# real-world-cryprography/APSU

Hardware: AMD Instinct MI355X
Metric: sender query-eval ms (ComputePowers + all BinBundles + gather), 16M-4096 params (lower is better)
Workload: dtype u64; 1 GPU; 16M-4096: n=8192, 4 bundle indices x 7 BinBundles (degrees [1303, 170]), 6 source -> 72 target powers, ps_low_degree=44; db_bytes_rank0=5459379072, binbundles_rank0=28, parallelism=binbundle-shard x1

## Files before the change

apsu_amd/csrc/engine_steps.cpp:

```cpp
#include "engine_impl.h"

#include <string>

namespace apsu_he {

namespace {

[[noreturn]] void refuse(const std::string &why) { throw std::invalid_argument("debug_run_step: " + why); }
void need(bool ok, const char *why) { if (!ok) refuse(why); }

void check_canonical(const u64 *x, size_t rows, const std::vector<u64> &mods, size_t n, const char *what)
{
    for (size_t r = 0; r < rows; r++) {
        const u64 m = mods[r % mods.size()], *row = x + r * n;
        u64 bad = 0;
        for (size_t k = 0; k < n; k++) bad |= (u64)(row[k] >= m);
        if (bad) refuse(std::string(what) + " holds a word that is not a canonical residue of its limb");
    }
}

}

void Engine::debug_run_step(const StepArgs &a)
{
    Enter g(this);
    TIER1_SLOTS();
    if (a.step == STEP_ROOTS_SPLIT) { debug_run_db_step(a); return; }
    if (a.step >= STEP_NTT_INFO) { debug_run_ntt_step(a); return; }
    if (a.step >= STEP_POLYN_WITH_ROOTS) { debug_run_db_step(a); return; }
    check_level(a.chain_idx);
    const LevelConstants &h = hlevel(a.chain_idx);
    const size_t n = hp_.n;
    const int L = h.L, nB = h.nB, nBsk = nB + 1, E = L + nBsk, K = hp_.K;
    const bool raw = a.flags & STEP_RAW, flag2 = a.flags & STEP_ACCUMULATE, store = a.flags & STEP_STORE, with_key = a.flags & STEP_KEY;
    const bool unrolled = behz_unrolled(L, nB);
    const std::vector<u64> q(h.q.begin(), h.q.end());
    std::vector<u64> bsk(h.B.begin(), h.B.end());
    bsk.push_back(h.m_sk);
    std::vector<u64> ext = q;
    ext.insert(ext.end(), bsk.begin(), bsk.end());
    const std::vector<u64> tmod{ hp_.t };
    const size_t batch = a.batch > 0 ? (size_t)a.batch : 0, polys = a.polys > 0 ? (size_t)a.polys : 0, terms = a.terms > 0 ? (size_t)a.terms : 0;

    if (a.step == STEP_LEVEL_INFO) {
        const size_t w = 4 + (size_t)L + nBsk + 2;
        need(a.out[0] && a.out_words[0] >= w, "level_info: out[0] too small");
        u64 *o = a.out[0];
        *o++ = (u64)L; *o++ = (u64)nB; *o++ = unrolled ? 1 : 0; *o++ = (u64)K;
        for (u64 v : q) *o++ = v;
        for (u64 v : bsk) *o++ = v;
        *o++ = hp_.using_keyswitching ? hp_.key_q[K - 1] : 0;
        *o++ = (u64)hp_.irrelevant_bit_count;
        return;
    }

    need(batch >= 1 && batch <= 64, "batch out of range (1 .. 64)");
    auto in_is = [&](int i, size_t words, const char *what) { if (!a.in[i] || a.in_words[i] != words) refuse(std::string(what) + ": wrong size"); };
    auto out_is = [&](int i, size_t words, const char *what) { if (!a.out[i] || a.out_words[i] != words) refuse(std::string(what) + ": wrong size"); };
    auto canon = [&](int i, const std::vector<u64> &mods, const char *what) { check_canonical(a.in[i], a.in_words[i] / n, mods, n, what); };
    auto canon_out = [&](int i, const std::vector<u64> &mods, const char *what) { check_canonical(a.out[i], a.out_words[i] / n, mods, n, what); };

    std::vector<FinishJob> fin;
    std::vector<FinishSumJob> fsum;
    std::vector<TensorJob> tj;
    std::vector<TensorConvJob> tcj;
    std::vector<TensorSumJob> tsj;
    std::vector<CtJob> cj;
    std::vector<SumJob> sj;
    std::vector<PlainJob> pj;
    std::vector<I0Job> ij;
    std::vector<EpiJob> ej;
    std::vector<unsigned char> flags8;

    WITH_ARENA({
        fin.clear(); fsum.clear(); tj.clear(); tcj.clear(); tsj.clear(); cj.clear(); sj.clear(); pj.clear(); ij.clear(); ej.clear();
        auto up = [&](const u64 *src, size_t words) {
            u64 *d = ws(words);
            HIP_CHECK(hipMemcpyAsync(d, src, words * sizeof(u64), hipMemcpyHostToDevice, st_));
            return d;
        };
        auto up_in = [&](int i) { return up(a.in[i], a.in_words[i]); };
        auto down = [&](int i, const u64 *src) { HIP_CHECK(hipMemcpyAsync(a.out[i], src, a.out_words[i] * sizeof(u64), hipMemcpyDeviceToHost, st_)); };
        auto jobs = [&](const auto &v) {
            using T = typename std::decay_t<decltype(v)>::value_type;
            T *d = ws_as<T>(v.size());
            HIP_CHECK(hipMemcpyAsync(d, v.data(), v.size() * sizeof(T), hipMemcpyHostToDevice, st_));
            return static_cast<const T *>(d);
        };

        switch (a.step) {
        case STEP_BEHZ_EXT: {
            need(polys >= 1 && polys <= 16, "behz_ext: polys out of range");
            need(!raw, "behz_ext: launch_behz_ext has no RAW form");
            in_is(0, batch * polys * L * n, "behz_ext: in[0] [batch][polys][L][n]");
            out_is(0, batch * polys * E * n, "behz_ext: out[0] [batch][polys][E][n]");
            canon(0, q, "behz_ext: in[0]");
            u64 *o = ws(a.out_words[0]);
            launch_behz_ext(dlevel(a.chain_idx), L, nB, up_in(0), polys * L * n, (int)polys, o, n, (int)batch, st_);
            down(0, o);
        } break;
        case STEP_DROP_BEHZ_EXT: {
            need(polys >= 1 && polys <= 16, "drop_behz_ext: polys out of range");
            need(a.chain_idx + 1 <= hp_.first_chain_idx, "drop_behz_ext: there is no level above chain_idx to drop from");
            need(unrolled, "drop_behz_ext: launch_drop_behz_ext exists for the unrolled sizes only (L == nB <= 3)");
            in_is(0, batch * polys * (L + 1) * n, "drop_behz_ext: in[0] [batch][polys][L + 1][n]");
            out_is(0, batch * polys * E * n, "drop_behz_ext: out[0] [batch][polys][E][n]");
            if (!raw) canon(0, hlevel(a.chain_idx + 1).q, "drop_behz_ext: in[0]");
            u64 *o = ws(a.out_words[0]);
            if (!launch_drop_behz_ext(dlevel(a.chain_idx), L, nB, up_in(0), polys * (L + 1) * n, (int)polys, o, n, (int)batch, st_, raw))
                throw std::logic_error("debug_run_step: launch_drop_behz_ext declined an unrolled level");
            down(0, o);
        } break;
        case STEP_TENSOR: {
            in_is(0, batch * 2 * E * n, "tensor: in[0] [batch][2][E][n]");
            in_is(1, batch * 2 * E * n, "tensor: in[1] [batch][2][E][n]");
            out_is(0, batch * 3 * E * n, "tensor: out[0] [batch][3][E][n]");
            canon(0, ext, "tensor: in[0]");
            canon(1, ext, "tensor: in[1]");
            const u64 *x = up_in(0), *y = up_in(1);
            u64 *o = ws(a.out_words[0]);
            for (size_t b = 0; b < batch; b++) tj.push_back(TensorJob{ x + b * 2 * E * n, y + b * 2 * E * n, o + b * 3 * E * n });
            launch_tensor(dlevel(a.chain_idx), jobs(tj), n, (int)batch, st_);
            down(0, o);
        } break;
        case STEP_TENSOR_CONV: {
            const size_t sa = polys, sb = terms;
            need(sa >= 1 && sb >= 1 && sa + sb - 1 <= CT_SIZE_MAX, "tensor_conv: sizes out of range (polys = sa, terms = sb, sa + sb - 1 <= 16)");
            in_is(0, batch * sa * E * n, "tensor_conv: in[0] [batch][sa][E][n]");
            in_is(1, batch * sb * E * n, "tensor_conv: in[1] [batch][sb][E][n]");
            out_is(0, batch * (sa + sb - 1) * E * n, "tensor_conv: out[0] [batch][sa + sb - 1][E][n]");
            canon(0, ext, "tensor_conv: in[0]");
            canon(1, ext, "tensor_conv: in[1]");
            const u64 *x = up_in(0), *y = up_in(1);
            u64 *o = ws(a.out_words[0]);
            for (size_t b = 0; b < batch; b++) tcj.push_back(TensorConvJob{ x + b * sa * E * n, y + b * sb * E * n, o + b * (sa + sb - 1) * E * n, (int)sa, (int)sb });
// ... 206 lines not shown
```

apsu_amd/csrc/kernels_behz.hip:

```cpp
#include "launch_behz.h"
#include "kernel_launch.h"
#include "eval_plan.h"

namespace apsu_he {

template <int TL, int TNB>
__global__ __launch_bounds__(EW_T) void k_behz_ext(const DevLevel *__restrict__ lv, const u64 *__restrict__ in,
                                                   size_t in_stride, int polys, u64 *__restrict__ out, size_t n)
{
    const size_t k = (size_t)blockIdx.x * EW_T + threadIdx.x;
    if (k >= n) return;
    const int L = TL ? TL : lv->L, nBsk = TL ? TNB + 1 : lv->nBsk, E = L + nBsk;
    constexpr int LMAX = TL ? TL : DMAXL;
    constexpr int BMAX = TL ? TNB + 1 : DMAXB;
    const size_t c = blockIdx.y / polys, p = blockIdx.y % polys;
    const u64 *src = in + c * in_stride + p * (size_t)L * n;
    u64 *dst = out + (size_t)blockIdx.y * E * n;
    u64 xs[LMAX];
    u32 mt_acc = 0;
#pragma unroll
    for (int j = 0; j < LMAX; j++) {
        if (TL || j < L) {
            const u64 x = src[(size_t)j * n + k];
            dst[(size_t)j * n + k] = x;
// ... 86 lines not shown
    }
    behz_ext2_body<TL>(lv, xin, dst, n, k);
}

bool launch_drop_behz_ext(const DevLevel *lv, int L, int nB, const u64 *in, size_t in_stride, int polys, u64 *out, size_t n, int cts,
                          hipStream_t st, bool raw)
{
    if (!cts) return true;
    const dim3 g = ew_grid(n, cts * polys), t(EW_T);
#define EXT2_CASE(TL) if (behz_unrolled(L, nB) && L == TL) { \
        if (raw) hipLaunchKernelGGL((k_behz_ext2<TL, true, true>), g, t, 0, st, lv, in, in_stride, polys, out, n); \
        else hipLaunchKernelGGL((k_behz_ext2<TL, true>), g, t, 0, st, lv, in, in_stride, polys, out, n); \
        KERNEL_CHECK(); return true; }
    EXT2_CASE(1) EXT2_CASE(2) EXT2_CASE(3)
#undef EXT2_CASE
    return false;
}

void launch_behz_ext(const DevLevel *lv, int L, int nB, const u64 *in, size_t in_stride, int polys, u64 *out, size_t n, int cts,
                     hipStream_t st)
{
    if (!cts) return;
    const dim3 g = ew_grid(n, cts * polys), t(EW_T);
#define EXT2_CASE(TL) if (behz_unrolled(L, nB) && L == TL) { hipLaunchKernelGGL((k_behz_ext2<TL, false>), g, t, 0, st, lv, in, in_stride, polys, out, n); KERNEL_CHECK(); return; }
    EXT2_CASE(1) EXT2_CASE(2) EXT2_CASE(3)
#undef EXT2_CASE
    if (L == 4 && nB == 4) hipLaunchKernelGGL((k_behz_ext<4, 4>), g, t, 0, st, lv, in, in_stride, polys, out, n);
    else hipLaunchKernelGGL((k_behz_ext<0, 0>), g, t, 0, st, lv, in, in_stride, polys, out, n);
    KERNEL_CHECK();
}

__global__ __launch_bounds__(EW_T) void k_tensor(const DevLevel *__restrict__ lv, const TensorJob *__restrict__ jobs, size_t n)
{
    const size_t k = (size_t)blockIdx.x * EW_T + threadIdx.x;
    if (k >= n) return;
    const TensorJob job = jobs[blockIdx.y];
    const int E = lv->E;
    const size_t ps = (size_t)E * n;
    for (int e = 0; e < E; e++) {
        const Mod m = lv->ext[e];
        const size_t o = e * n + k;
        const u64 a0 = job.a[o], a1 = job.a[ps + o], b0 = job.b[o], b1 = job.b[ps + o];
        job.d[o] = mulmod(a0, b0, m);
        u128p mid = mul128(a0, b1);
        mac128(mid, a1, b0);
        job.d[ps + o] = barrett128(mid, m);
        job.d[2 * ps + o] = mulmod(a1, b1, m);
    }
}

void launch_tensor(const DevLevel *lv, const TensorJob *jobs, size_t n, int batch, hipStream_t st)
{
    hipLaunchKernelGGL(k_tensor, ew_grid(n, batch), dim3(EW_T), 0, st, lv, jobs, n);
    KERNEL_CHECK();
}

__global__ __launch_bounds__(EW_T) void k_tensor_conv(const DevLevel *__restrict__ lv, const TensorConvJob *__restrict__ jobs, size_t n)
{
    const size_t k = (size_t)blockIdx.x * EW_T + threadIdx.x;
    if (k >= n) return;
    const TensorConvJob job = jobs[blockIdx.y];
    const int E = lv->E;
    const size_t ps = (size_t)E * n;
    const int so = job.sa + job.sb - 1;
    for (int e = 0; e < E; e++) {
        const Mod m = lv->ext[e];
        const size_t o = e * n + k;
        for (int I = 0; I < so; I++) {
            const int i0 = I - (job.sb - 1) > 0 ? I - (job.sb - 1) : 0, i1 = I < job.sa - 1 ? I : job.sa - 1;
            u64 acc = 0;
            for (int i = i0; i <= i1; i++) acc = addmod(acc, mulmod(job.a[i * ps + o], job.b[(I - i) * ps + o], m), m.q);
            job.d[I * ps + o] = acc;
        }
    }
}

void launch_tensor_conv(const DevLevel *lv, const TensorConvJob *jobs, size_t n, int njobs, hipStream_t st)
{
    if (!njobs) return;
    hipLaunchKernelGGL(k_tensor_conv, ew_grid(n, njobs), dim3(EW_T), 0, st, lv, jobs, n);
    KERNEL_CHECK();
}

__global__ __launch_bounds__(EW_T) void k_tensor_sum(const DevLevel *__restrict__ lv, const TensorSumJob *__restrict__ jobs, size_t n, int e0)
{
    const size_t k = (size_t)blockIdx.x * EW_T + threadIdx.x;
    if (k >= n) return;
    const TensorSumJob job = jobs[blockIdx.z];
    const int E = lv->E, L = lv->L, e = blockIdx.y + e0;
    const size_t ps = (size_t)E * n, o = (size_t)e * n + k;
    const Mod m = lv->ext[e];
    if (e < L) {
        for (int i = 0; i < job.terms; i++) {
            const u64 *a = job.a + (size_t)i * 2 * ps, *b = job.b + (size_t)i * 2 * ps;
            const u64 a0 = a[o], a1 = a[ps + o], b0 = b[o], b1 = b[ps + o];
            u64 *d = job.dq + (size_t)i * 3 * L * n + o;
            d[0] = mulmod(a0, b0, m);
            u128p mid = mul128(a0, b1);
            mac128(mid, a1, b0);
            d[(size_t)L * n] = barrett128(mid, m);
            d[(size_t)2 * L * n] = mulmod(a1, b1, m);
        }
    } else {
        u128p s0{ 0, 0 }, s1{ 0, 0 }, s2{ 0, 0 };
        u64 r0 = 0, r1 = 0, r2 = 0;
        for (int i = 0; i < job.terms; i++) {
            const u64 *a = job.a + (size_t)i * 2 * ps, *b = job.b + (size_t)i * 2 * ps;
            const u64 a0 = a[o], a1 = a[ps + o], b0 = b[o], b1 = b[ps + o];
            mac128(s0, a0, b0);
            mac128(s1, a0, b1);
            mac128(s1, a1, b0);
            mac128(s2, a1, b1);
            if ((i & 7) == 7 || i + 1 == job.terms) {
                r0 = addmod(r0, barrett128(s0, m), m.q);
                r1 = addmod(r1, barrett128(s1, m), m.q);
                r2 = addmod(r2, barrett128(s2, m), m.q);
                s0 = s1 = s2 = u128p{ 0, 0 };
            }
        }
        const int nBsk = E - L;
        u64 *d = job.bs + (size_t)(e - L) * n + k;
        d[0] = r0;
        d[(size_t)nBsk * n] = r1;
        d[(size_t)2 * nBsk * n] = r2;
    }
}

void launch_tensor_sum(const DevLevel *lv, int E, const TensorSumJob *jobs, size_t n, int njobs, int e0, hipStream_t st)
{
    if (!njobs || e0 >= E) return;
    hipLaunchKernelGGL(k_tensor_sum, dim3((unsigned)((n + EW_T - 1) / EW_T), E - e0, njobs), dim3(EW_T), 0, st, lv, jobs, n, e0);
    KERNEL_CHECK();
}

template <int TL, int TNB>
__device__ __forceinline__ void behz_finish_coeff(const DevLevel *__restrict__ lv, const u64 *__restrict__ dq, size_t term_stride,
                                                  int terms, const u64 *__restrict__ dbsk, size_t n, u64 *res )
{
    const int L = TL ? TL : lv->L, nB = TL ? TNB : lv->nB, nBsk = nB + 1;
    constexpr int LMAX = TL ? TL : DMAXL;
    constexpr int BMAX = TL ? TNB + 1 : DMAXB;
    u64 xq[LMAX];
#pragma unroll
    for (int j = 0; j < LMAX; j++) xq[j] = 0;
    for (int it = 0; it < terms; it++) {
#pragma unroll
        for (int j = 0; j < LMAX; j++)
            if (TL || j < L) xq[j] += mul_shoup(dq[it * term_stride + (size_t)j * n], lv->t_inv_punct_q[j].w, lv->t_inv_punct_q[j].wq, lv->q[j].q);
    }
    u64 ys[BMAX];
    u64 fl_sk = 0;
#pragma unroll
    for (int i = 0; i < BMAX; i++) {
        if (TL || i < nBsk) {
            const Mod m = lv->bsk[i];
            u128p acc{ 0, 0 };
#pragma unroll
            for (int j = 0; j < LMAX; j++)
                if (TL || j < L) mac128(acc, xq[j], lv->q_to_bsk[i][j]);
            const u64 conv = barrett128(acc, m);
            const u64 xb = mul_shoup(dbsk[(size_t)i * n], lv->t_bsk[i].w, lv->t_bsk[i].wq, m.q);
            const u64 fl = mul_shoup(xb + (m.q - conv), lv->inv_prod_q_bsk[i].w, lv->inv_prod_q_bsk[i].wq, m.q);
            if (i < nB) ys[i] = mul_shoup(fl, lv->inv_punct_B[i].w, lv->inv_punct_B[i].wq, m.q);
            else fl_sk = fl;
        }
    }
    const Mod msk = lv->bsk[nB];
    u128p acc{ 0, 0 };
#pragma unroll
    for (int i = 0; i < BMAX - 1; i++)
        if (TL || i < nB) mac128(acc, ys[i], lv->B_to_msk[i]);
    const u64 z_sk = barrett128(acc, msk);
    const u64 alpha = mul_shoup(z_sk + (msk.q - fl_sk), lv->inv_prod_B_msk.w, lv->inv_prod_B_msk.wq, msk.q);
    const bool neg = alpha > lv->msk_half;
    const u64 a_abs = neg ? msk.q - alpha : alpha;
#pragma unroll
    for (int j = 0; j < LMAX; j++) {
        if (TL || j < L) {
            u128p z{ 0, 0 };
#pragma unroll
            for (int i = 0; i < BMAX - 1; i++)
                if (TL || i < nB) mac128(z, ys[i], lv->B_to_q[j][i]);
            mac128(z, a_abs, neg ? lv->prod_B_q[j] : lv->neg_prod_B_q[j]);
            res[j] = barrett128(z, lv->q[j]);
        }
    }
}

template <int TL, int TNB>
__global__ __launch_bounds__(EW_T) void k_behz_finish(const DevLevel *__restrict__ lv, const FinishJob *__restrict__ jobs,
                                                      int accumulate, size_t n)
{
    const size_t k = (size_t)blockIdx.x * EW_T + threadIdx.x;
    if (k >= n) return;
    const int L = TL ? TL : lv->L, E = TL ? 2 * TL + 1 + (TNB - TL) : lv->E;
    constexpr int LMAX = TL ? TL : DMAXL;
    const FinishJob job = jobs[blockIdx.y / 3];
    const size_t p = blockIdx.y % 3;
    u64 sum[LMAX];
    u64 *o = job.out + p * (size_t)L * n + k;
#pragma unroll
    for (int j = 0; j < LMAX; j++)
        if (TL || j < L) sum[j] = accumulate ? o[(size_t)j * n] : 0;
    for (int i = 0; i < job.terms; i++) {
        const u64 *dp = job.d + (((size_t)i * 3 + p) * (size_t)E) * n + k;
        u64 res[LMAX];
        behz_finish_coeff<TL, TNB>(lv, dp, 0, 1, dp + (size_t)L * n, n, res);
#pragma unroll
        for (int j = 0; j < LMAX; j++)
            if (TL || j < L) sum[j] = addmod(sum[j], res[j], lv->q[j].q);
    }
#pragma unroll
    for (int j = 0; j < LMAX; j++)
        if (TL || j < L) o[(size_t)j * n] = sum[j];
}

#if defined(__HIP_DEVICE_COMPILE__) && !defined(APSU_FIN_NO_FENCE)
#define FIN_LOAD_FENCE() asm volatile("" ::: "memory")
#else
#define FIN_LOAD_FENCE() do { } while (0)
#endif
template <int TL>
__device__ __forceinline__ void behz_finish_coeff2(const DevLevel *__restrict__ lv, const u64 *__restrict__ dq, size_t term_stride,
                                                   int terms, const u64 *__restrict__ dbsk, size_t n, u64 *res, size_t kidx)
{
    constexpr int L = TL, nB = TL, nBsk = TL + 1;
    u64 xq[L];
#pragma unroll
    for (int j = 0; j < L; j++) xq[j] = 0;
    ShoupConst cq[L];
#pragma unroll
    for (int j = 0; j < L; j++) { const u64x2 v = ldg16(reinterpret_cast<const u64 *>(lv->fin_q[j] + kidx)); cq[j] = ShoupConst{ v[0], v[1] }; }
    for (int it = 0; it < terms; it++) {
#pragma unroll
        for (int j = 0; j < L; j++)
            xq[j] += mul_shoup(dq[it * term_stride + (size_t)j * n], cq[j].w, cq[j].wq, lv->q[j].q);
    }
    u64 ys[nB];
    u64 fl_sk = 0;
#pragma unroll
    for (int i = 0; i < nBsk; i++) {
        FIN_LOAD_FENCE();
        const u64 m = lv->bsk[i].q;
        u64 conv = 0;
#pragma unroll
        for (int j = 0; j < L; j++) conv += lazy2(xq[j], lv->s_q_to_bsk[i][j], m);
        const u64x2 cb = ldg16(reinterpret_cast<const u64 *>(lv->fin_b[i] + kidx));
        const u64 xb = lazy2(dbsk[(size_t)i * n], ShoupConst{ cb[0], cb[1] }, m);
        const u64 diff = xb + ((u64)(2 * L) * m - conv);
        const u64 f = mul_shoup(diff, lv->s_fl[i].w, lv->s_fl[i].wq, m);
        if (i < nB) ys[i] = f; else fl_sk = f;
    }
    const u64 msk = lv->bsk[nB].q;
    u64 z_sk = msk - fl_sk;
#pragma unroll
    for (int i = 0; i < nB; i++) z_sk += lazy2(ys[i], lv->s_B_to_msk[i], msk);
    const u64 alpha = mul_shoup(z_sk, lv->inv_prod_B_msk.w, lv->inv_prod_B_msk.wq, msk);
    const bool neg = alpha > lv->msk_half;
    const u64 a_abs = neg ? msk - alpha : alpha;
#pragma unroll
    for (int j = 0; j < L; j++) {
        FIN_LOAD_FENCE();
        const u64 q = lv->q[j].q;
        u64 z = lazy2(a_abs, neg ? lv->s_prod_B_q[j] : lv->s_neg_prod_B_q[j], q);
#pragma unroll
        for (int i = 0; i < nB; i++) z += lazy2(ys[i], lv->s_B_to_q[j][i], q);
        res[j] = csub(csub(csub(z, q << 2), q << 1), q);
    }
}

template <int TL>
__global__ __launch_bounds__(EW_T) void k_behz_finish2(const DevLevel *__restrict__ lv, const FinishJob *__restrict__ jobs,
                                                       int accumulate, size_t n)
{
    const size_t k = (size_t)blockIdx.x * EW_T + threadIdx.x;
    if (k >= n) return;
    constexpr int L = TL, E = 2 * TL + 1;
    const FinishJob job = jobs[blockIdx.y / 3];
    const size_t p = blockIdx.y % 3;
    u64 sum[L];
    u64 *o = job.out + p * (size_t)L * n + k;
#pragma unroll
    for (int j = 0; j < L; j++) sum[j] = accumulate ? o[(size_t)j * n] : 0;
    for (int i = 0; i < job.terms; i++) {
        u64 res[L];
        const u64 *dp = job.d + (((size_t)i * 3 + p) * (size_t)E) * n + k;
        behz_finish_coeff2<TL>(lv, dp, 0, 1, dp + (size_t)L * n, n, res, k);
#pragma unroll
        for (int j = 0; j < L; j++) sum[j] = addmod(sum[j], res[j], lv->q[j].q);
    }
#pragma unroll
    for (int j = 0; j < L; j++) o[(size_t)j * n] = sum[j];
}

void launch_behz_finish(const DevLevel *lv, int L, int nB, const FinishJob *jobs, bool accumulate, size_t n, int njobs, hipStream_t st)
{
    if (!njobs) return;
    const dim3 g = ew_grid(n, njobs * 3), t(EW_T);
    const int acc = accumulate ? 1 : 0;
#define FIN2_CASE(TL) if (behz_unrolled(L, nB) && L == TL) { hipLaunchKernelGGL((k_behz_finish2<TL>), g, t, 0, st, lv, jobs, acc, n); KERNEL_CHECK(); return; }
    FIN2_CASE(1) FIN2_CASE(2) FIN2_CASE(3)
#undef FIN2_CASE
    if (L == 4 && nB == 4) hipLaunchKernelGGL((k_behz_finish<4, 4>), g, t, 0, st, lv, jobs, acc, n);
    else hipLaunchKernelGGL((k_behz_finish<0, 0>), g, t, 0, st, lv, jobs, acc, n);
    KERNEL_CHECK();
}

template <int TL, bool LAZY>
__global__ __launch_bounds__(EW_T) void k_behz_finish_sum(const DevLevel *__restrict__ lv, const FinishSumJob *__restrict__ jobs, size_t n)
{
    const size_t k = (size_t)blockIdx.x * EW_T + threadIdx.x;
    if (k >= n) return;
    const int L = TL ? TL : lv->L, nBsk = TL ? TL + 1 : lv->nBsk;
    constexpr int LMAX = TL ? TL : DMAXL;
    const FinishSumJob job = jobs[blockIdx.y / 3];
    const size_t p = blockIdx.y % 3;
    const u64 *dq = job.dq + p * (size_t)L * n + k;
    const u64 *db = job.bs + p * (size_t)nBsk * n + k;
    u64 res[LMAX];
    if constexpr (LAZY) behz_finish_coeff2<TL>(lv, dq, (size_t)3 * L * n, job.terms, db, n, res, k);
// ... 117 lines not shown
    KERNEL_CHECK();
}

template <bool MD>
__global__ __launch_bounds__(EW_T) void k_eval_epilogue(const DevLevel *__restrict__ levels, int lvl, const EpiJob *__restrict__ jobs,
                                                        size_t ct_poly_stride, u64 clear_mask, size_t n, const DevKey *__restrict__ key)
{
    const size_t k = (size_t)blockIdx.x * EW_T + threadIdx.x;
    if (k >= n) return;
    const EpiJob job = jobs[blockIdx.y];
    const DevLevel *lv = levels + lvl;
    const int L = lvl + 1;
    u64 v[2][DMAXL];
#pragma unroll
    for (int p = 0; p < 2; p++) {
        u64 tl = 0;
        const u64 *a = nullptr;
        if constexpr (MD) {
            a = job.ks_acc + (size_t)p * (L + 1) * n;
            const Mod pm = key->q[key->K - 1];
            const u64x2 tw = ldg16(reinterpret_cast<const u64 *>(key->p_tw + k));
            tl = barrett64(mul_shoup(a[(size_t)L * n + k], tw[0], tw[1], pm.q) + key->p_half, pm);
        }
#pragma unroll
        for (int j = 0; j < DMAXL; j++)
            if (j < L) {
                const u64 q = lv->q[j].q;
                u64 x = job.ct[p * ct_poly_stride + (size_t)j * n + k];
                if constexpr (MD) {
                    const Mod m = key->q[j];
                    const u64 tk = submod(barrett64(tl, m), key->p_half_mod[j], m.q);
                    const u64x2 tw = ldg16(reinterpret_cast<const u64 *>(key->md_tw[j] + k));
                    const u64 u = mul_shoup_lazy(a[(size_t)j * n + k], tw[0], tw[1], m.q);
                    const u64 w = mul_shoup_lazy(tk, key->inv_p[j].w, key->inv_p[j].wq, m.q);
                    x = addmod(x, csub(csub(u + (m.q << 1) - w, m.q << 1), m.q), m.q);
                }
                if (job.add1) x = addmod(x, job.add1[((size_t)p * L + j) * n + k], q);
                if (job.add2) x = addmod(x, job.add2[((size_t)p * L + j) * n + k], q);
                v[p][j] = x;
            }
    }
    {
        const u64 m0 = job.a0[k], m1 = job.mask[k];
        const u64 f0 = plain_fix(lv, m0), f1 = plain_fix(lv, m1);
#pragma unroll
        for (int j = 0; j < DMAXL; j++)
            if (j < L) {
                const u64 q = lv->q[j].q;
                v[0][j] = addmod(addmod(v[0][j], scaled_plain(lv, m0, f0, j), q), scaled_plain(lv, m1, f1, j), q);
            }
    }
    for (int l = lvl; l > 0; l--) {
        const DevLevel *ll = levels + l;
        const u64 ql = ll->q[l].q;
#pragma unroll
        for (int p = 0; p < 2; p++) {
            u64 last = 0;
#pragma unroll
            for (int j = 0; j < DMAXL; j++) if (j == l) last = v[p][j];
            last = addmod(last, ll->half, ql);
#pragma unroll
            for (int j = 0; j < DMAXL; j++)
                if (j < l) {
                    const Mod m = ll->q[j];
                    const u64 tmp = submod(barrett64(last, m), ll->half_mod[j], m.q);
                    v[p][j] = mul_shoup(submod(v[p][j], tmp, m.q), ll->inv_q_last[j].w, ll->inv_q_last[j].wq, m.q);
                }
        }
    }
    job.out[k] = v[0][0] & clear_mask;
    job.out[n + k] = v[1][0] & clear_mask;
}

void launch_eval_epilogue(const DevLevel *levels, int lvl, const EpiJob *jobs, size_t ct_poly_stride, int clear_bits, size_t n,
                          int njobs, hipStream_t st, const DevKey *key)
{
    if (!njobs) return;
    const u64 mask = clear_bits > 0 ? ~(((u64)1 << clear_bits) - 1) : ~(u64)0;
    if (key) hipLaunchKernelGGL(k_eval_epilogue<true>, ew_grid(n, njobs), dim3(EW_T), 0, st, levels, lvl, jobs, ct_poly_stride, mask, n, key);
    else hipLaunchKernelGGL(k_eval_epilogue<false>, ew_grid(n, njobs), dim3(EW_T), 0, st, levels, lvl, jobs, ct_poly_stride, mask, n, key);
    KERNEL_CHECK();
}

template <bool RAW>
__global__ __launch_bounds__(EW_T) void k_i0_finish(const DevLevel *__restrict__ lv, const I0Job *__restrict__ jobs, size_t n)
{
    const size_t k = (size_t)blockIdx.x * EW_T + threadIdx.x;
    if (k >= n) return;
    const I0Job job = jobs[blockIdx.y >> 1];
    const int p = blockIdx.y & 1;
    const int L = lv->L;
    const u64 ql = lv->q[L - 1].q, half = lv->half;
    u64 R = 0;
    const u64 *v = job.v + (size_t)p * n + k;
    u64 tw0 = 0, tw1 = 0;
    if (RAW) { const u64x2 tw = ldg16(reinterpret_cast<const u64 *>(lv->last_tw + k)); tw0 = tw[0]; tw1 = tw[1]; }
    for (int t = 0; t < job.terms; t++) {
        u64 x = v[(size_t)t * 2 * n];
        if (RAW) x = mul_shoup(x, tw0, tw1, ql);
        R += addmod(x, half, ql);
    }
    for (int m = 0; m + 1 < L; m++) {
        const Mod mq = lv->q[m];
        const u64 th = barrett128(mul128((u64)job.terms, lv->half_mod[m]), mq);
        const u64 corr = submod(th, barrett64(R, mq), mq.q);
        const size_t o = ((size_t)p * (L - 1) + m) * n + k;
        u64 r;
        if (RAW) {
            const u64x2 tw = ldg16(reinterpret_cast<const u64 *>(lv->drop_tw[m] + k));
            const u64 a = mul_shoup_lazy(job.s[o], tw[0], tw[1], mq.q);
            const u64 b = mul_shoup_lazy(corr, lv->inv_q_last[m].w, lv->inv_q_last[m].wq, mq.q);
            r = csub(csub(a + b, mq.q << 1), mq.q);
        } else {
            const u64 val = addmod(job.s[o], corr, mq.q);
            r = mul_shoup(val, lv->inv_q_last[m].w, lv->inv_q_last[m].wq, mq.q);
        }
        job.acc[o] = job.store ? r : addmod(job.acc[o], r, mq.q);
    }
}

void launch_i0_finish(const DevLevel *lv_low, const I0Job *jobs, size_t n, int njobs, hipStream_t st, bool raw)
{
    if (!njobs) return;
    if (raw) hipLaunchKernelGGL(k_i0_finish<true>, ew_grid(n, njobs * 2), dim3(EW_T), 0, st, lv_low, jobs, n);
    else hipLaunchKernelGGL(k_i0_finish<false>, ew_grid(n, njobs * 2), dim3(EW_T), 0, st, lv_low, jobs, n);
    KERNEL_CHECK();
}

}
```

apsu_amd/csrc/launch_behz.h:

```cpp
#pragma once
#include <hip/hip_runtime.h>
#include "dev_consts.h"
#include "launch_ntt.h"

namespace apsu_he {

void launch_behz_ext(const DevLevel *lv, int L, int nB, const u64 *in, size_t in_stride, int polys, u64 *out, size_t n, int cts,
                     hipStream_t st);
bool launch_drop_behz_ext(const DevLevel *lv, int L, int nB, const u64 *in, size_t in_stride, int polys, u64 *out, size_t n, int cts,
                          hipStream_t st, bool raw = false);
void launch_tensor(const DevLevel *lv, const TensorJob *jobs, size_t n, int batch, hipStream_t st);
struct TensorConvJob { const u64 *a, *b; u64 *d; int sa, sb; };
void launch_tensor_conv(const DevLevel *lv, const TensorConvJob *jobs, size_t n, int njobs, hipStream_t st);
struct TensorSumJob { const u64 *a, *b; u64 *dq, *bs; int terms; int pad; };
void launch_tensor_sum(const DevLevel *lv, int E, const TensorSumJob *jobs, size_t n, int njobs, int e0, hipStream_t st);
struct FinishSumJob { const u64 *dq, *bs; u64 *out; int terms; int pad; };
void launch_behz_finish_sum(const DevLevel *lv, int L, int nB, const FinishSumJob *jobs, size_t n, int njobs, hipStream_t st);
struct FinishJob { const u64 *d; u64 *out; int terms; int pad; };
void launch_behz_finish(const DevLevel *lv, int L, int nB, const FinishJob *jobs, bool accumulate, size_t n, int njobs, hipStream_t st);
void launch_ks_inner(const DevKey *key, int L, const u64 *tdec, const u64 *rk, u64 *acc, size_t n, int batch,
                     hipStream_t st);
void launch_ks_moddown(const DevKey *key, int L, const u64 *acc, u64 *ct, size_t ct_stride, size_t n, int batch,
                       hipStream_t st, const DevLevel *lv = nullptr, u64 *ext = nullptr, int n_ext = 0, bool raw = false);
struct EpiJob { const u64 *ct; const u64 *add1; const u64 *add2; const u64 *a0; const u64 *mask; u64 *out;
                const u64 *ks_acc = nullptr; };
void launch_eval_epilogue(const DevLevel *levels, int lvl, const EpiJob *jobs, size_t ct_poly_stride, int clear_bits, size_t n,
                          int njobs, hipStream_t st, const DevKey *key = nullptr);
struct I0Job { const u64 *s; const u64 *v; u64 *acc; int terms; int store; };
void launch_i0_finish(const DevLevel *lv_low, const I0Job *jobs, size_t n, int njobs, hipStream_t st, bool raw = false);

}
```

apsu_amd/csrc/modmath.h:

```cpp
#pragma once
#include <stdint.h>

#if defined(__HIPCC__)
#include <hip/hip_runtime.h>
#define HD __host__ __device__ __forceinline__
#else
#define HD inline
#endif

typedef uint64_t u64;
typedef uint32_t u32;

#if defined(__clang__)
typedef u64 u64x2 __attribute__((ext_vector_type(2), __may_alias__));
#else
typedef u64 u64x2 __attribute__((vector_size(16), __may_alias__));
#endif

HD u64x2 ldg16(const u64 *p)
{
#if defined(__HIP_DEVICE_COMPILE__)
    return *(const u64x2 __attribute__((address_space(1))) *)(const void *)p;
#else
    return *reinterpret_cast<const u64x2 *>(p);
#endif
}
HD u64x2 ldg16_nt(const u64 *p)
{
#if defined(__HIP_DEVICE_COMPILE__)
    return __builtin_nontemporal_load((const u64x2 __attribute__((address_space(1))) *)(const void *)p);
#else
    return *reinterpret_cast<const u64x2 *>(p);
#endif
}

#if defined(__clang__)
typedef u32 u32x4a4 __attribute__((ext_vector_type(4), __may_alias__, aligned(4)));
#else
typedef u32 u32x4a4 __attribute__((vector_size(16), __may_alias__, aligned(4)));
#endif
HD u32x4a4 ldg16_a4_nt(const u32 *p)
{
#if defined(__HIP_DEVICE_COMPILE__)
    return __builtin_nontemporal_load((const u32x4a4 __attribute__((address_space(1))) *)(const void *)p);
#else
    return *reinterpret_cast<const u32x4a4 *>(p);
#endif
}

struct u128p { u64 lo, hi; };

HD u64 mulhi64(u64 a, u64 b)
{
#if defined(__HIP_DEVICE_COMPILE__)
    return __umul64hi(a, b);
#else
    return (u64)(((unsigned __int128)a * b) >> 64);
#endif
}

HD u128p mul128(u64 a, u64 b) { return { a * b, mulhi64(a, b) }; }

HD void add128(u128p &acc, u128p x)
{
    u64 lo = acc.lo + x.lo;
    acc.hi += x.hi + (lo < acc.lo);
    acc.lo = lo;
}

HD void mac128(u128p &acc, u64 a, u64 b) { add128(acc, mul128(a, b)); }

struct Mod {
    u64 q;
    u64 r0, r1;
};

HD u64 barrett128(u128p x, const Mod &m)
{
    u64 carry = mulhi64(x.lo, m.r0);
    u128p t2 = mul128(x.lo, m.r1);
    u64 tmp1 = t2.lo + carry;
    u64 tmp3 = t2.hi + (tmp1 < carry);
    t2 = mul128(x.hi, m.r0);
    u64 s = tmp1 + t2.lo;
    carry = t2.hi + (s < tmp1);
    u64 qhat = x.hi * m.r1 + tmp3 + carry;
    u64 r = x.lo - qhat * m.q;
    return r >= m.q ? r - m.q : r;
}

HD u64 barrett64(u64 x, const Mod &m)
{
    u64 r = x - mulhi64(x, m.r1) * m.q;
    return r >= m.q ? r - m.q : r;
}

HD u64 mulmod(u64 a, u64 b, const Mod &m) { return barrett128(mul128(a, b), m); }

HD u64 addmod(u64 a, u64 b, u64 q) { u64 s = a + b; return s >= q ? s - q : s; }
HD u64 submod(u64 a, u64 b, u64 q) { return a >= b ? a - b : a + q - b; }

HD u64 mul_shoup_lazy(u64 x, u64 w, u64 wq, u64 q) { return x * w - mulhi64(x, wq) * q; }

HD u64 mul_shoup(u64 x, u64 w, u64 wq, u64 q)
{
    u64 r = mul_shoup_lazy(x, w, wq, q);
    return r >= q ? r - q : r;
}

HD u64 csub(u64 x, u64 q) { return x >= q ? x - q : x; }
```

apsu_amd/engine.py:

```python
import collections
import ctypes as C
import json
import os

import numpy as np

_HERE = os.path.dirname(os.path.abspath(__file__))
_LIB = None
u64p = C.POINTER(C.c_uint64)


class ApsuHeError(RuntimeError):
    pass


class _Info(C.Structure):
    _fields_ = [
        ("poly_modulus_degree", C.c_uint64), ("plain_modulus", C.c_uint64),
        ("coeff_modulus_size", C.c_int32), ("first_chain_idx", C.c_int32),
        ("using_keyswitching", C.c_int32), ("irrelevant_bit_count", C.c_int32),
        ("coeff_modulus", C.c_uint64 * 8),
        ("ps_low_degree", C.c_uint32), ("max_items_per_bin", C.c_uint32),
        ("bundle_idx_count", C.c_uint32), ("items_per_bundle", C.c_uint32),
        ("source_power_count", C.c_uint32), ("target_power_count", C.c_uint32),
# ... 349 lines not shown
        _check(load_library().apsu_he_relinearize(self.h, _p(work), rk.h, chain_idx))
        return np.ascontiguousarray(work[:2])

    def mod_switch_to_next(self, ct, chain_idx):
        work = np.ascontiguousarray(ct.copy())
        polys = ct.shape[0]
        _check(load_library().apsu_he_mod_switch_to_next(self.h, _p(work), polys, chain_idx))
        return np.ascontiguousarray(work.reshape(-1)[: polys * chain_idx * self.n].reshape(polys, chain_idx, self.n))

    def clear_irrelevant_bits(self, ct):
        _check(load_library().apsu_he_clear_irrelevant_bits(self.h, _p(ct), ct.shape[0]))

    def upload_relin_keys(self, rk):
        h = C.c_void_p()
        _check(load_library().apsu_he_relin_upload(self.h, _p(np.ascontiguousarray(rk)), C.byref(h)))
        return RelinKeys(self, h)

    def upload_bundle(self, bundle_idx, cache_idx, coeffs, is_ntt):
        h = C.c_void_p()
        flags = (C.c_uint8 * len(coeffs))(*[1 if f else 0 for f in is_ntt])
        keep = [np.ascontiguousarray(c, dtype=np.uint64) for c in coeffs]
        _check(load_library().apsu_he_db_upload_bundle(self.h, bundle_idx, cache_idx, len(keep), _ptr_array(keep), flags,
                                                       C.byref(h)))
        return Bundle(self, h, bundle_idx, cache_idx, len(keep) - 1)

    def build_bundle(self, bundle_idx, cache_idx, bins):
        nb = len(bins)
        stride = max([len(b) for b in bins] + [1])
        roots = np.zeros((max(nb, 1), stride), dtype=np.uint64)
        counts = np.zeros(max(nb, 1), dtype=np.uint32)
        for i, b in enumerate(bins):
            counts[i] = len(b)
            roots[i, :len(b)] = b
        h = C.c_void_p()
        _check(load_library().apsu_he_db_build_bundle(self.h, bundle_idx, cache_idx, _p(roots), C.c_void_p(counts.ctypes.data),
                                                      nb, stride, C.byref(h)))
        deg = C.c_uint32()
        _check(load_library().apsu_he_bundle_degree(h, C.byref(deg)))
        return Bundle(self, h, bundle_idx, cache_idx, deg.value)

    def update_bundle(self, bundle, inserts=None, removes=None):
        args, keep, nb = _update_lists(inserts, removes)
        h = C.c_void_p()
        _check(load_library().apsu_he_bundle_update(self.h, bundle.h, *args, nb, C.byref(h)))
        deg = C.c_uint32()
        _check(load_library().apsu_he_bundle_degree(h, C.byref(deg)))
        return Bundle(self, h, bundle.bundle_idx, bundle.cache_idx, deg.value)

    def bin_counts(self, bundle):
        counts = np.empty(self.n, dtype=np.uint32)
        _check(load_library().apsu_he_bundle_bin_counts(self.h, bundle.h, C.c_void_p(counts.ctypes.data)))
        return counts

    def bins(self, bundle, _form=0):
        lib = load_library()
        counts = np.empty(self.n, dtype=np.uint32)
        _check(lib.apsu_he_bundle_bin_counts(self.h, bundle.h, C.c_void_p(counts.ctypes.data)))
        stride = _bins_stride(counts)
        roots = np.zeros((self.n, stride), dtype=np.uint64)
        if _form:
            _check(lib.apsu_he_debug_bundle_bins_form(self.h, bundle.h, _p(roots), C.c_void_p(counts.ctypes.data), C.c_uint32(stride), C.c_int(_form)))
        else:
            _check(lib.apsu_he_bundle_bins(self.h, bundle.h, _p(roots), C.c_void_p(counts.ctypes.data), C.c_uint32(stride)))
        return _bins_list(roots, counts)

    def debug_run_step(self, step, chain_idx, ins=(), outs=(), flags=0, terms=0, polys=0, batch=1, e0=0, n_ext=0):
        a = _StepArgs()
        a.step, a.chain_idx, a.flags = STEPS[step], chain_idx, flags
        a.terms, a.polys, a.batch, a.e0, a.n_ext = terms, polys, batch, e0, n_ext
        for i, x in enumerate(ins):
            if x is not None:
                a.inp[i], a.in_words[i] = _p(x), x.size
        for i, x in enumerate(outs):
            if x is not None:
                a.out[i], a.out_words[i] = _p(x), x.size
        _check(load_library().apsu_he_debug_run_step(self.h, C.byref(a)))

    def level_info(self, chain_idx):
        out = np.zeros(64, dtype=np.uint64)
        self.debug_run_step("level_info", chain_idx, outs=[out])
        v = [int(x) for x in out]
        L, nB = v[0], v[1]
        return dict(L=L, nB=nB, unrolled=bool(v[2]), K=v[3], q=v[4:4 + L], B=v[4 + L:4 + L + nB], m_sk=v[4 + L + nB], p=v[5 + L + nB],
                    clear_bits=v[6 + L + nB])

    def eval_plain(self, bundles, x, masks=None, want_is_bin=False):
        count = len(bundles)
        x = np.ascontiguousarray(x, dtype=np.uint64).reshape(count, self.n)
        if masks is not None:
            masks = np.ascontiguousarray(masks, dtype=np.uint64).reshape(count, self.n)
        out = np.empty((count, self.n), dtype=np.uint64)
        is_bin = np.zeros((count, self.n), dtype=np.uint8) if want_is_bin else None
        hs = (C.c_void_p * count)(*[b.h for b in bundles])
        _check(load_library().apsu_he_bundles_eval_plain(self.h, hs, C.c_uint32(count), _p(x), 0, _p(masks) if masks is not None else None, 0,
                                                         _p(out), 0, C.c_void_p(is_bin.ctypes.data) if want_is_bin else None))
        return (out, is_bin.astype(bool)) if want_is_bin else out

    def eval_plain_times(self):
        a, b, c = C.c_double(), C.c_double(), C.c_double()
        _check(load_library().apsu_he_debug_eval_plain_times(self.h, C.byref(a), C.byref(b), C.byref(c)))
        return a.value, b.value, c.value

    def self_test(self, bundles, seed=None, x=None):
        sd = self._seed_words(seed)
        count = len(bundles)
        hs = (C.c_void_p * max(count, 1))(*[b.h for b in bundles])
        if x is not None:
            x = np.ascontiguousarray(x, dtype=np.uint64)
            if x.size != len({b.bundle_idx for b in bundles}) * self.n:
                raise ValueError("x must hold n slot values per distinct bundle index")
        rep = _SelfTestReport()
        _check(load_library().apsu_he_db_self_test(self.h, hs, C.c_uint32(count), _p(sd), _p(x) if x is not None else None, C.byref(rep)))
        return _self_test_report(rep)

    def self_test_times(self):
        ms = (C.c_double * 5)()
        _check(load_library().apsu_he_debug_self_test_times(self.h, ms))
        return tuple(float(v) for v in ms)

    def bins_times(self):
        a, b, c = C.c_double(), C.c_double(), C.c_double()
        _check(load_library().apsu_he_debug_bins_times(self.h, C.byref(a), C.byref(b), C.byref(c)))
        return a.value, b.value, c.value

    def lookup(self, bundles, entries):
        felts, start = _entries(entries, self.felts_per_item)
        present = np.zeros((len(bundles), len(start)), dtype=np.uint8)
        room = np.zeros((len(bundles), len(start)), dtype=np.uint32)
        hs = (C.c_void_p * max(len(bundles), 1))(*[b.h for b in bundles])
        _check(load_library().apsu_he_bundles_lookup(self.h, hs, len(bundles), _p(felts), C.c_void_p(start.ctypes.data), C.c_size_t(len(start)),
                                                     C.c_void_p(present.ctypes.data), C.c_void_p(room.ctypes.data)))
        return present.astype(bool), room

    def lookup_times(self):
        a, k = C.c_double(), C.c_double()
        _check(load_library().apsu_he_debug_lookup_times(self.h, C.byref(a), C.byref(k)))
        return a.value, k.value

    def apply_entries(self, bundles, inserts=None, removes=None, bundle_idx=None):
        if bundle_idx is None:
            if not bundles:
                raise ValueError("apply_entries: bundle_idx is needed when no BinBundle is given")
            bundle_idx = bundles[0].bundle_idx
        fi, si = _entries(inserts, self.felts_per_item)
        fr, sr = _entries(removes, self.felts_per_item)
        nb = len(bundles)
        hs = (C.c_void_p * max(nb, 1))(*[b.h for b in bundles])
        state = np.zeros(nb, dtype=np.uint32)
        replaced = (C.c_void_p * max(nb, 1))()
        appended = (C.c_void_p * max(len(si), 1))()
        n_app = C.c_uint32()
        out = [np.zeros(len(si), dtype=np.uint32), np.zeros(len(si), dtype=np.uint32), np.zeros(len(sr), dtype=np.uint32), np.zeros(len(sr), dtype=np.uint32)]
        u32 = lambda a: C.c_void_p(a.ctypes.data)
        L = load_library()
        _check(L.apsu_he_db_apply_entries(self.h, C.c_uint32(bundle_idx), hs, nb, _p(fi), u32(si), C.c_size_t(len(si)), _p(fr), u32(sr), C.c_size_t(len(sr)),
                                          u32(state), replaced, appended, C.byref(n_app), *[u32(a) for a in out]))

        def wrap(h, bundle_idx, cache_idx):
            h = C.c_void_p(h)
            deg = C.c_uint32()
            _check(L.apsu_he_bundle_degree(h, C.byref(deg)))
            return Bundle(self, h, bundle_idx, cache_idx, deg.value)
        news = [wrap(replaced[i], b.bundle_idx, b.cache_idx) if replaced[i] else None for i, b in enumerate(bundles)]
        first = bundles[-1].cache_idx + 1 if bundles else 0
        apps = [wrap(appended[k], bundle_idx, first + k) for k in range(n_app.value)]
        return ApplyResult(state, news, apps, *out)

# ... 614 lines not shown
```

Baseline: 3.175 ms.

## Vectorize and batch term loads in tensor-sum, BEHZ finish and i0-finish kernels

k_tensor_sum and k_i0_finish now handle two coefficients per thread with 16-byte loads and stores, and fetch groups of terms up front behind a scheduling barrier so more memory requests are in flight. The BEHZ finish sum over term residues issues grouped nontemporal loads when the level shape is static. Together these target latency-bound strided loads in the memory-heavy reduction kernels. In exchange they raise register pressure, halve the thread count, and add tail handling for term counts that do not fill a group.

```diff
diff --git a/apsu_amd/csrc/engine_steps.cpp b/apsu_amd/csrc/engine_steps.cpp
--- a/apsu_amd/csrc/engine_steps.cpp
+++ b/apsu_amd/csrc/engine_steps.cpp
@@ -43,7 +43,7 @@
     const size_t batch = a.batch > 0 ? (size_t)a.batch : 0, polys = a.polys > 0 ? (size_t)a.polys : 0, terms = a.terms > 0 ? (size_t)a.terms : 0;
 
     if (a.step == STEP_LEVEL_INFO) {
-        const size_t w = 4 + (size_t)L + nBsk + 2;
+        const size_t w = 4 + (size_t)L + nBsk + 2 + 3;
         need(a.out[0] && a.out_words[0] >= w, "level_info: out[0] too small");
         u64 *o = a.out[0];
         *o++ = (u64)L; *o++ = (u64)nB; *o++ = unrolled ? 1 : 0; *o++ = (u64)K;
@@ -51,6 +51,7 @@
         for (u64 v : bsk) *o++ = v;
         *o++ = hp_.using_keyswitching ? hp_.key_q[K - 1] : 0;
         *o++ = (u64)hp_.irrelevant_bit_count;
+        *o++ = (u64)TENSOR_SUM_GROUP; *o++ = (u64)finish_sum_group(L, nB); *o++ = (u64)I0_FINISH_GROUP;
         return;
     }
 
diff --git a/apsu_amd/csrc/kernels_behz.hip b/apsu_amd/csrc/kernels_behz.hip
--- a/apsu_amd/csrc/kernels_behz.hip
+++ b/apsu_amd/csrc/kernels_behz.hip
@@ -192,55 +192,142 @@
     KERNEL_CHECK();
 }
 
+#if defined(__HIP_DEVICE_COMPILE__)
+#define GROUP_LOADS_ISSUED() __builtin_amdgcn_sched_barrier(0)
+#else
+#define GROUP_LOADS_ISSUED() do { } while (0)
+#endif
+constexpr int TS_U = TENSOR_SUM_GROUP;
+static_assert(8 % TS_U == 0, "a group of k_tensor_sum must not straddle a fold of its 128-bit sums");
 __global__ __launch_bounds__(EW_T) void k_tensor_sum(const DevLevel *__restrict__ lv, const TensorSumJob *__restrict__ jobs, size_t n, int e0)
 {
-    const size_t k = (size_t)blockIdx.x * EW_T + threadIdx.x;
+    const size_t k = ((size_t)blockIdx.x * EW_T + threadIdx.x) * 2;
     if (k >= n) return;
     const TensorSumJob job = jobs[blockIdx.z];
-    const int E = lv->E, L = lv->L, e = blockIdx.y + e0;
+    const int E = lv->E, L = lv->L, e = blockIdx.y + e0, terms = job.terms;
     const size_t ps = (size_t)E * n, o = (size_t)e * n + k;
     const Mod m = lv->ext[e];
+    const u64 *a = job.a + o, *b = job.b + o;
+    u64x2 a0[TS_U], a1[TS_U], b0[TS_U], b1[TS_U];
+    auto load_group = [&](int i) {
+#pragma unroll
+        for (int u = 0; u < TS_U; u++) {
+            const size_t t = (size_t)(i + u < terms ? i + u : terms - 1) * 2 * ps;
+            a0[u] = ldg16_nt(a + t), a1[u] = ldg16_nt(a + t + ps), b0[u] = ldg16(b + t), b1[u] = ldg16(b + t + ps);
+        }
+        GROUP_LOADS_ISSUED();
+    };
     if (e < L) {
-        for (int i = 0; i < job.terms; i++) {
-            const u64 *a = job.a + (size_t)i * 2 * ps, *b = job.b + (size_t)i * 2 * ps;
-            const u64 a0 = a[o], a1 = a[ps + o], b0 = b[o], b1 = b[ps + o];
-            u64 *d = job.dq + (size_t)i * 3 * L * n + o;
-            d[0] = mulmod(a0, b0, m);
-            u128p mid = mul128(a0, b1);
-            mac128(mid, a1, b0);
-            d[(size_t)L * n] = barrett128(mid, m);
-            d[(size_t)2 * L * n] = mulmod(a1, b1, m);
+        auto product = [&](int i, int u) {
+            u64 d0[2], d1[2], d2[2];
+#pragma unroll
+            for (int c = 0; c < 2; c++) {
+                d0[c] = mulmod(a0[u][c], b0[u][c], m);
+                u128p mid = mul128(a0[u][c], b1[u][c]);
+                mac128(mid, a1[u][c], b0[u][c]);
+                d1[c] = barrett128(mid, m);
+                d2[c] = mulmod(a1[u][c], b1[u][c], m);
+            }
+            u64 *d = job.dq + (size_t)(i + u) * 3 * L * n + o;
+            stg16(d, d0[0], d0[1]);
+            stg16(d + (size_t)L * n, d1[0], d1[1]);
+            stg16(d + (size_t)2 * L * n, d2[0], d2[1]);
+        };
+        int i = 0;
+        for (; i + TS_U <= terms; i += TS_U) {
+            load_group(i);
+#pragma unroll
+            for (int u = 0; u < TS_U; u++) product(i, u);
+        }
+        if (i < terms) {
+            load_group(i);
+#pragma unroll
+            for (int u = 0; u < TS_U; u++)
+                if (i + u < terms) product(i, u);
         }
     } else {
-        u128p s0{ 0, 0 }, s1{ 0, 0 }, s2{ 0, 0 };
-        u64 r0 = 0, r1 = 0, r2 = 0;
-        for (int i = 0; i < job.terms; i++) {
-            const u64 *a = job.a + (size_t)i * 2 * ps, *b = job.b + (size_t)i * 2 * ps;
-            const u64 a0 = a[o], a1 = a[ps + o], b0 = b[o], b1 = b[ps + o];
-            mac128(s0, a0, b0);
-            mac128(s1, a0, b1);
-            mac128(s1, a1, b0);
-            mac128(s2, a1, b1);
-            if ((i & 7) == 7 || i + 1 == job.terms) {
-                r0 = addmod(r0, barrett128(s0, m), m.q);
-                r1 = addmod(r1, barrett128(s1, m), m.q);
-                r2 = addmod(r2, barrett128(s2, m), m.q);
-                s0 = s1 = s2 = u128p{ 0, 0 };
+        u128p s[2][3] = {};
+        auto add_term = [&](int u) {
+#pragma unroll
+            for (int c = 0; c < 2; c++) {
+                mac128w(s[c][0], a0[u][c], b0[u][c]);
+                mac128w(s[c][1], a0[u][c], b1[u][c]);
+                mac128w(s[c][1], a1[u][c], b0[u][c]);
+                mac128w(s[c][2], a1[u][c], b1[u][c]);
             }
-        }
+        };
+        auto fold = [&]() {
+#pragma unroll
+            for (int c = 0; c < 2; c++)
+#pragma unroll
+                for (int x = 0; x < 3; x++) s[c][x] = u128p{ barrett128(s[c][x], m), 0 };
+        };
+        int i = 0;
+        for (; i + TS_U <= terms; i += TS_U) {
+            load_group(i);
+#pragma unroll
+            for (int u = 0; u < TS_U; u++) add_term(u);
+            if (((i + TS_U) & 7) == 0) fold();
+        }
+        if (i < terms) {
+            load_group(i);
+#pragma unroll
+            for (int u = 0; u < TS_U; u++)
+                if (i + u < terms) add_term(u);
+        }
+        if (terms & 7) fold();
         const int nBsk = E - L;
         u64 *d = job.bs + (size_t)(e - L) * n + k;
-        d[0] = r0;
-        d[(size_t)nBsk * n] = r1;
-        d[(size_t)2 * nBsk * n] = r2;
+#pragma unroll
+        for (int x = 0; x < 3; x++) stg16(d + (size_t)x * nBsk * n, s[0][x].lo, s[1][x].lo);
     }
 }
 
 void launch_tensor_sum(const DevLevel *lv, int E, const TensorSumJob *jobs, size_t n, int njobs, int e0, hipStream_t st)
 {
     if (!njobs || e0 >= E) return;
-    hipLaunchKernelGGL(k_tensor_sum, dim3((unsigned)((n + EW_T - 1) / EW_T), E - e0, njobs), dim3(EW_T), 0, st, lv, jobs, n, e0);
-    KERNEL_CHECK();
+    hipLaunchKernelGGL(k_tensor_sum, dim3((unsigned)((n / 2 + EW_T - 1) / EW_T), E - e0, njobs), dim3(EW_T), 0, st, lv, jobs, n, e0);
+    KERNEL_CHECK();
+}
+
+template <int LMAX, bool STATIC, class F>
+__device__ __forceinline__ void sum_term_residues(const u64 *__restrict__ dq, size_t term_stride, int terms, size_t n, int L, u64 *xq, F scale)
+{
+    constexpr int U = STATIC ? finish_sum_group(LMAX, LMAX) : 1;
+    if (terms == 1) {
+#pragma unroll
+        for (int j = 0; j < LMAX; j++)
+            if (STATIC || j < L) xq[j] += scale(j, dq[(size_t)j * n]);
+        return;
+    }
+    if (!STATIC) {
+        for (int it = 0; it < terms; it++) {
+#pragma unroll
+            for (int j = 0; j < LMAX; j++)
+                if (j < L) xq[j] += scale(j, dq[it * term_stride + (size_t)j * n]);
+        }
+        return;
+    }
+    auto group = [&](int it, auto full) {
+        constexpr bool FULL = decltype(full)::value;
+        const u64 *p[U];
+#pragma unroll
+        for (int u = 0; u < U; u++) p[u] = dq + (size_t)(FULL || it + u < terms ? it + u : terms - 1) * term_stride;
+        u64 x[LMAX][U];
+#pragma unroll
+        for (int j = 0; j < LMAX; j++)
+#pragma unroll
+            for (int u = 0; u < U; u++) x[j][u] = ldg8_nt(p[u] + (size_t)j * n);
+        GROUP_LOADS_ISSUED();
+#pragma unroll
+        for (int j = 0; j < LMAX; j++)
+#pragma unroll
+            for (int u = 0; u < U; u++)
+                if (FULL || it + u < terms) xq[j] += scale(j, x[j][u]);
+    };
+    int it = 0;
+    for (; it + U <= terms; it += U) group(it, std::true_type{});
+    if (it < terms) group(it, std::false_type{});
 }
 
 template <int TL, int TNB>
@@ -253,11 +340,9 @@
     u64 xq[LMAX];
 #pragma unroll
     for (int j = 0; j < LMAX; j++) xq[j] = 0;
-    for (int it = 0; it < terms; it++) {
-#pragma unroll
-        for (int j = 0; j < LMAX; j++)
-            if (TL || j < L) xq[j] += mul_shoup(dq[it * term_stride + (size_t)j * n], lv->t_inv_punct_q[j].w, lv->t_inv_punct_q[j].wq, lv->q[j].q);
-    }
+    sum_term_residues<LMAX, TL != 0>(dq, term_stride, terms, n, L, xq, [&](int j, u64 x) {
+        return mul_shoup(x, lv->t_inv_punct_q[j].w, lv->t_inv_punct_q[j].wq, lv->q[j].q);
+    });
     u64 ys[BMAX];
     u64 fl_sk = 0;
 #pragma unroll
@@ -341,11 +426,9 @@
     ShoupConst cq[L];
 #pragma unroll
     for (int j = 0; j < L; j++) { const u64x2 v = ldg16(reinterpret_cast<const u64 *>(lv->fin_q[j] + kidx)); cq[j] = ShoupConst{ v[0], v[1] }; }
-    for (int it = 0; it < terms; it++) {
-#pragma unroll
-        for (int j = 0; j < L; j++)
-            xq[j] += mul_shoup(dq[it * term_stride + (size_t)j * n], cq[j].w, cq[j].wq, lv->q[j].q);
-    }
+    sum_term_residues<L, true>(dq, term_stride, terms, n, L, xq, [&](int j, u64 x) {
+        return mul_shoup(x, cq[j].w, cq[j].wq, lv->q[j].q);
+    });
     u64 ys[nB];
     u64 fl_sk = 0;
 #pragma unroll
@@ -629,49 +712,73 @@
     KERNEL_CHECK();
 }
 
+constexpr int I0_U = I0_FINISH_GROUP;
 template <bool RAW>
 __global__ __launch_bounds__(EW_T) void k_i0_finish(const DevLevel *__restrict__ lv, const I0Job *__restrict__ jobs, size_t n)
 {
-    const size_t k = (size_t)blockIdx.x * EW_T + threadIdx.x;
+    const size_t k = ((size_t)blockIdx.x * EW_T + threadIdx.x) * 2;
     if (k >= n) return;
     const I0Job job = jobs[blockIdx.y >> 1];
-    const int p = blockIdx.y & 1;
+    const int p = blockIdx.y & 1, terms = job.terms;
     const int L = lv->L;
     const u64 ql = lv->q[L - 1].q, half = lv->half;
-    u64 R = 0;
+    u64 R[2] = { 0, 0 };
     const u64 *v = job.v + (size_t)p * n + k;
-    u64 tw0 = 0, tw1 = 0;
-    if (RAW) { const u64x2 tw = ldg16(reinterpret_cast<const u64 *>(lv->last_tw + k)); tw0 = tw[0]; tw1 = tw[1]; }
-    for (int t = 0; t < job.terms; t++) {
-        u64 x = v[(size_t)t * 2 * n];
-        if (RAW) x = mul_shoup(x, tw0, tw1, ql);
-        R += addmod(x, half, ql);
-    }
+    u64x2 ltw[2] = {};
+    if (RAW) { ltw[0] = ldg16(reinterpret_cast<const u64 *>(lv->last_tw + k)); ltw[1] = ldg16(reinterpret_cast<const u64 *>(lv->last_tw + k + 1)); }
+    auto group = [&](int t, auto full) {
+        constexpr bool FULL = decltype(full)::value;
+        u64x2 x[I0_U];
+#pragma unroll
+        for (int u = 0; u < I0_U; u++) x[u] = ldg16_nt(v + (size_t)(FULL || t + u < terms ? t + u : terms - 1) * 2 * n);
+        GROUP_LOADS_ISSUED();
+#pragma unroll
+        for (int u = 0; u < I0_U; u++)
+            if (FULL || t + u < terms) {
+#pragma unroll
+                for (int c = 0; c < 2; c++) {
+                    u64 y = x[u][c];
+                    if (RAW) y = mul_shoup(y, ltw[c][0], ltw[c][1], ql);
+                    R[c] += addmod(y, half, ql);
+                }
+            }
+    };
+    int t = 0;
+    for (; t + I0_U <= terms; t += I0_U) group(t, std::true_type{});
+    if (t < terms) group(t, std::false_type{});
     for (int m = 0; m + 1 < L; m++) {
         const Mod mq = lv->q[m];
-        const u64 th = barrett128(mul128((u64)job.terms, lv->half_mod[m]), mq);
-        const u64 corr = submod(th, barrett64(R, mq), mq.q);
+        const u64 th = barrett128(mul128((u64)terms, lv->half_mod[m]), mq);
         const size_t o = ((size_t)p * (L - 1) + m) * n + k;
-        u64 r;
-        if (RAW) {
-            const u64x2 tw = ldg16(reinterpret_cast<const u64 *>(lv->drop_tw[m] + k));
-            const u64 a = mul_shoup_lazy(job.s[o], tw[0], tw[1], mq.q);
-            const u64 b = mul_shoup_lazy(corr, lv->inv_q_last[m].w, lv->inv_q_last[m].wq, mq.q);
-            r = csub(csub(a + b, mq.q << 1), mq.q);
-        } else {
-            const u64 val = addmod(job.s[o], corr, mq.q);
-            r = mul_shoup(val, lv->inv_q_last[m].w, lv->inv_q_last[m].wq, mq.q);
-        }
-        job.acc[o] = job.store ? r : addmod(job.acc[o], r, mq.q);
+        const u64x2 s = ldg16(job.s + o);
+        u64x2 acc = {};
+        if (!job.store) acc = ldg16(job.acc + o);
+        u64 r[2];
+#pragma unroll
+        for (int c = 0; c < 2; c++) {
+            const u64 corr = submod(th, barrett64(R[c], mq), mq.q);
+            if (RAW) {
+                const u64x2 tw = ldg16(reinterpret_cast<const u64 *>(lv->drop_tw[m] + k + c));
+                const u64 a = mul_shoup_lazy(s[c], tw[0], tw[1], mq.q);
+                const u64 b = mul_shoup_lazy(corr, lv->inv_q_last[m].w, lv->inv_q_last[m].wq, mq.q);
+                r[c] = csub(csub(a + b, mq.q << 1), mq.q);
+            } else {
+                const u64 val = addmod(s[c], corr, mq.q);
+                r[c] = mul_shoup(val, lv->inv_q_last[m].w, lv->inv_q_last[m].wq, mq.q);
+            }
+            if (!job.store) r[c] = addmod(acc[c], r[c], mq.q);
+        }
+        stg16(job.acc + o, r[0], r[1]);
     }
 }
 
 void launch_i0_finish(const DevLevel *lv_low, const I0Job *jobs, size_t n, int njobs, hipStream_t st, bool raw)
 {
     if (!njobs) return;
-    if (raw) hipLaunchKernelGGL(k_i0_finish<true>, ew_grid(n, njobs * 2), dim3(EW_T), 0, st, lv_low, jobs, n);
-    else hipLaunchKernelGGL(k_i0_finish<false>, ew_grid(n, njobs * 2), dim3(EW_T), 0, st, lv_low, jobs, n);
-    KERNEL_CHECK();
-}
-
-}
+    const dim3 g = ew_grid(n / 2, njobs * 2);
+    if (raw) hipLaunchKernelGGL(k_i0_finish<true>, g, dim3(EW_T), 0, st, lv_low, jobs, n);
+    else hipLaunchKernelGGL(k_i0_finish<false>, g, dim3(EW_T), 0, st, lv_low, jobs, n);
+    KERNEL_CHECK();
+}
+
+}
diff --git a/apsu_amd/csrc/launch_behz.h b/apsu_amd/csrc/launch_behz.h
--- a/apsu_amd/csrc/launch_behz.h
+++ b/apsu_amd/csrc/launch_behz.h
@@ -4,6 +4,10 @@
 #include "launch_ntt.h"
 
 namespace apsu_he {
+
+constexpr int TENSOR_SUM_GROUP = 2;
+constexpr int I0_FINISH_GROUP = 8;
+constexpr int finish_sum_group(int L, int nB) { return L == nB && L <= 4 ? 4 : 1; }
 
 void launch_behz_ext(const DevLevel *lv, int L, int nB, const u64 *in, size_t in_stride, int polys, u64 *out, size_t n, int cts,
                      hipStream_t st);
diff --git a/apsu_amd/csrc/modmath.h b/apsu_amd/csrc/modmath.h
--- a/apsu_amd/csrc/modmath.h
+++ b/apsu_amd/csrc/modmath.h
@@ -23,6 +23,23 @@
     return *(const u64x2 __attribute__((address_space(1))) *)(const void *)p;
 #else
     return *reinterpret_cast<const u64x2 *>(p);
+#endif
+}
+HD u64 ldg8_nt(const u64 *p)
+{
+#if defined(__HIP_DEVICE_COMPILE__)
+    return __builtin_nontemporal_load((const u64 __attribute__((address_space(1))) *)(const void *)p);
+#else
+    return *p;
+#endif
+}
+HD void stg16(u64 *p, u64 v0, u64 v1)
+{
+#if defined(__HIP_DEVICE_COMPILE__)
+    *(u64x2 __attribute__((address_space(1))) *)(void *)p = u64x2{ v0, v1 };
+#else
+    p[0] = v0;
+    p[1] = v1;
 #endif
 }
 HD u64x2 ldg16_nt(const u64 *p)
@@ -70,6 +87,13 @@
 
 HD void mac128(u128p &acc, u64 a, u64 b) { add128(acc, mul128(a, b)); }
 
+HD void mac128w(u128p &acc, u64 a, u64 b)
+{
+    const unsigned __int128 s = ((unsigned __int128)acc.hi << 64 | acc.lo) + (unsigned __int128)a * b;
+    acc.lo = (u64)s;
+    acc.hi = (u64)(s >> 64);
+}
+
 struct Mod {
     u64 q;
     u64 r0, r1;
diff --git a/apsu_amd/engine.py b/apsu_amd/engine.py
--- a/apsu_amd/engine.py
+++ b/apsu_amd/engine.py
@@ -455,7 +455,7 @@
         v = [int(x) for x in out]
         L, nB = v[0], v[1]
         return dict(L=L, nB=nB, unrolled=bool(v[2]), K=v[3], q=v[4:4 + L], B=v[4 + L:4 + L + nB], m_sk=v[4 + L + nB], p=v[5 + L + nB],
-                    clear_bits=v[6 + L + nB])
+                    clear_bits=v[6 + L + nB], groups=tuple(v[7 + L + nB:10 + L + nB]))
 
     def eval_plain(self, bundles, x, masks=None, want_is_bin=False):
         count = len(bundles)
```

Measured after the change: 3.142 ms (median of 6 runs). -1.0%, faster.
